# fatchord/WaveRNN

Measured on AMD Instinct MI355X. Metric: audio samples/sec (real-time factor @22.05 kHz), MoL WaveRNN batched generate, higher is better.
Workload: dtype f32

## Files before the change

### wavernn_amd/csrc/wrnn_duo.hip

```cpp
#include <type_traits>

#include "wrnn_ring.h"

namespace wrnn {

#ifndef DUO_XR_FIRST
#define DUO_XR_FIRST 1
#endif

#ifndef DUO_ABLATE
#define DUO_ABLATE 0
#endif
#ifndef DUO_EI_DEPTH
#define DUO_EI_DEPTH 4
#endif

constexpr int DNWGC = 4 * LNJ;
#ifndef DUO_GH_SHIFT
#define DUO_GH_SHIFT 1
#endif
constexpr int DLOGS = 36;
constexpr int DPART = 2 * NW * 3 * 256;
static_assert(O_HOWN == 768 && O_XS == 1024 && O_SP == 1040, "saved state layout");

struct DuoLds {
    int off_h, off_seg, off_xs, off_part, off_log, off_misc, off_prof, off_f3, total;
};
__host__ __device__ inline DuoLds duo_lds(int G)
{
    DuoLds l;
    int o = 0;
    l.off_h = o;    o += G * 256;
    l.off_seg = o;  o += G * 48;
    l.off_xs = o;   o += G * 16;
    l.off_part = o; o += DPART;
    l.off_log = o;  o += SEG * DLOGS;
    l.off_misc = o; o += 2 * LMAXG + 2 * DNWGC;
    l.off_prof = o; o += 2 * 16;
    o = (o + 3) & ~3;
    l.off_f3 = o;   o += SEG * LDC;
    l.total = o;
    return l;
}

#define DPARTOF(q) (PART + (q) * (NW * 3 * 256))
#define PHX(k)                                                                 \
    do {                                                                       \
        if (PROF && tid == 0) {                                                \
            const u64 now_ = __builtin_amdgcn_s_memtime();                     \
            PROFL[k] += now_ - plast;                                          \
            plast = now_;                                                      \
            if (trp && t >= tr_t0 && t < tr_t0 + 3 && ntr < 510)               \
                trp[1 + ntr++] = (now_ << 16) | (u64)(((tri & 15) << 8) | ((k) & 255));   \
        }                                                                      \
    } while (0)
#define TRACE_DECL                                                                                                   \
    u64 *const trp = (PROF && (a.tuning & 16384) && a.prof) ? a.prof + 256 * 32 + (size_t)blockIdx.x * 512 : nullptr; \
    int ntr = 0, tri = 0;                                                                                            \
    const int tr_t0 = a.t0 + (a.t1 - a.t0) / 2;

typedef __attribute__((address_space(3))) void lds_void;
__device__ __forceinline__ void prefetch8(__amdgpu_buffer_rsrc_t rs, float *dst, int voff, int soff)
{
    lds_void *d0 = (lds_void *)dst, *d1 = (lds_void *)(dst + 1024);
    __builtin_amdgcn_raw_ptr_buffer_load_lds(rs, d0, 16, voff, soff, 0, 16 );
    __builtin_amdgcn_raw_ptr_buffer_load_lds(rs, d0, 16, voff, soff, 1024, 16);
    __builtin_amdgcn_raw_ptr_buffer_load_lds(rs, d0, 16, voff, soff, 2048, 16);
    __builtin_amdgcn_raw_ptr_buffer_load_lds(rs, d0, 16, voff, soff, 3072, 16);
    __builtin_amdgcn_raw_ptr_buffer_load_lds(rs, d1, 16, voff + 4096, soff, 0, 16);
    __builtin_amdgcn_raw_ptr_buffer_load_lds(rs, d1, 16, voff + 4096, soff, 1024, 16);
    __builtin_amdgcn_raw_ptr_buffer_load_lds(rs, d1, 16, voff + 4096, soff, 2048, 16);
    __builtin_amdgcn_raw_ptr_buffer_load_lds(rs, d1, 16, voff + 4096, soff, 3072, 16);
}

struct DuoGeo {
    int nact;
    u64 nbpack;
};

template <int MODE, bool LA, bool LP, bool EI, bool PROF>
__device__ __forceinline__ void duo_ih(const LoopArgs &a, float *smem, const int cl, const int J, const int ncl, const bool loc_h, const bool loc_y)
{
    const int G = a.G;
    const DuoLds L = duo_lds(G);
    float *HS = smem + L.off_h, *XS = smem + L.off_xs, *PART = smem + L.off_part;
    int *SEGT = reinterpret_cast<int *>(smem + L.off_seg);
    int *GEO = reinterpret_cast<int *>(smem + L.off_misc);
    u64 *PROFL = reinterpret_cast<u64 *>(smem + L.off_prof);
    u64 plast = 0;
    TRACE_DECL
    const int tid = threadIdx.x, lane = tid & 63, w = __builtin_amdgcn_readfirstlane(tid >> 6);
    const int fi = lane & 15, kq = lane >> 4;
    const int kbase_lane = KCH * w + 4 * kq;
    const int pu = 4 * w + (tid & 3), pj = (tid >> 2) & 15;
    const int prow = LU * J + pu;
    const int T0 = a.t0, T1 = a.t1;
    const int NR = a.Btot, NGR = a.NG;
    unsigned *const status = a.status;
    float *const state = a.state;
    u64 *const profp = a.prof;
    const float *const bhhp = LA ? a.b_hh1 : a.b_hh2;
    const int resume = a.resume, hop = a.hop;
    const int zrow = a.Nall * a.tab_fps;
    constexpr int L_H = LA ? 0 : 1, L_XR = LA ? 5 : 6, L_Y = LA ? 2 : 3, L_GH = LA ? 8 : 12;
    constexpr int L_P0 = LA ? 4 : 5, L_P2 = LA ? 6 : 2;

    float A_ih[3][AF], A_fc[AF];
#pragma unroll
    for (int g = 0; g < 3; ++g) load_afrag(A_ih[g], LA ? a.w_ih1 : a.w_ih2, LA ? H : H + AUX, g * H + LU * J + fi, true, kbase_lane);
    load_afrag(A_fc, LA ? a.fc1_w : a.fc2_w, H + AUX, LU * J + fi, true, kbase_lane);
    float cb_r = 0.f, cb_z = 0.f, cb_n = 0.f, ux_r = 0.f, ux_z = 0.f, ux_n = 0.f, w0o = 0.f;
    if constexpr (LA) {
        cb_r = a.b_ih1[prow]; cb_z = a.b_ih1[H + prow]; cb_n = a.b_ih1[2 * H + prow];
        ux_r = a.u1[prow]; ux_z = a.u1[H + prow]; ux_n = a.u1[2 * H + prow];
        w0o = a.I_w0[prow];
    }

    for (int q = tid; q < L.total; q += NT) smem[q] = 0.f;
    __syncthreads();
    DuoGeo geo;
    geo.nact = 0; geo.nbpack = 0;
    const size_t state_wg = ((size_t)(cl * LNWGC + 2 * J + (LA ? 0 : 1)) * G) * LGRP;
    for (int i = 0; i < G; ++i) {
        const int g = cl + ncl * i;
        if (g >= NGR) break;
        geo.nact = i + 1;
        const int b0 = (int)(((long)g * NR) / NGR), nb = (int)(((long)(g + 1) * NR) / NGR) - b0;
        if (tid == 0) { GEO[2 * i] = a.rb0 + b0; GEO[2 * i + 1] = nb; }
        geo.nbpack |= (u64)(unsigned)nb << (8 * i);
        if (a.resume) {
            const float *sg = a.state + state_wg + (size_t)i * LGRP;
            HS[i * 256 + tid] = sg[O_HOWN + tid];
            if (tid < SEG) XS[i * 16 + tid] = sg[O_XS + tid];
            if (tid < 2 * SEG) SEGT[i * 48 + tid] = reinterpret_cast<const int *>(sg + O_SP)[tid];
        } else if (tid < SEG) {
            const int sc = a.rb0 + b0 + (tid < nb ? tid : nb - 1);
            SEGT[i * 48 + tid] = a.seg_pos[sc];
            SEGT[i * 48 + SEG + tid] = a.seg_lim[sc];
        }
    }
    __syncthreads();
    for (int i = 0; i < geo.nact; ++i) {
        if (tid < SEG) {
            const int nb = (int)((geo.nbpack >> (8 * i)) & 255u);
            const int sc = GEO[2 * i] + (tid < nb ? tid : nb - 1);
            SEGT[i * 48 + 2 * SEG + tid] = sc * a.tab_fps - (SEGT[i * 48 + tid] + a.tab_t0) / a.hop;
        }
    }
    __syncthreads();
    const int nact = geo.nact;
    const u64 nbpack = geo.nbpack;

    const __amdgpu_buffer_rsrc_t xrs = make_rsrc(a.xbuf, (unsigned)(DXBUF_FLOATS * 4));
    const __amdgpu_buffer_rsrc_t crs = make_rsrc(a.c2f, 0x7FFFF000u);
    const __amdgpu_buffer_rsrc_t frs = make_rsrc(LA ? a.c3f : a.c4f, 0x7FFFF000u);
    const int voff_frag = frag_off(w, 0, lane) * 4;
    const int voff_own = (((J * 64) + 16 * w + pj) * 4 + (tid & 3)) * 4;
    const int voff_gh = (256 * (J & 7) + tid) * 16;
    const int cbase = cl * DSLOTB;
    const unsigned magic = a.hop_magic;
    const int mshift = a.hop_shift;

    const int locbits = (loc_h ? 1 : 0) | (loc_y ? 2 : 0);
    const bool late_xo = (a.tuning & 128) == 0, reprobe = (a.tuning & 8) == 0;
    const bool full_chk = !PROF && (a.tuning & 4096) != 0;
    bool dead = false;
    int pp = 0;
    int t = T0;
    int cur = 0;

    struct Carry {
        float c0, c1, c2;
        u32x4 gw;
        unsigned xo, xt;
        int i, pp, t;
    };
    Carry cy;
    cy.c0 = cy.c1 = cy.c2 = 0.f; cy.gw = u32x4{0u, 0u, 0u, 0u}; cy.xo = cy.xt = 0u; cy.i = 0; cy.pp = 0; cy.t = T0;

    auto slot_nb = [&](int i) -> int { return (int)((nbpack >> (8 * i)) & 255u); };

    auto back_gates = [&](const Carry &c) {
        const int bi = c.i, bt = c.t;
        const float *PB = DPARTOF(c.pp);
        const int nb = slot_nb(bi);
        const int sb = cbase + bi * (MAXCL * DSLOTB) + (bt & (DRING - 1)) * XTB;
        const bool live = pj < nb;
        lds_barrier();
        PHX(cur + 1);
        const float pr = get_partial<3>(PB, 0, pu, pj), pz = get_partial<3>(PB, 1, pu, pj), pn = get_partial<3>(PB, 2, pu, pj);
        const float hprev = HS[bi * 256 + tid];
        float ghr, ghz, ghn;
        u32x4 g = c.gw;
        if (bt > T0) {
            const unsigned tag = (unsigned)bt + 1u;
            if (__builtin_expect(__any(live && g.w != tag), 0))
                wait_for([&] { return !__any(live && g.w != tag); },
                         [&] { g = __builtin_amdgcn_raw_buffer_load_b128(xrs, voff_gh, cbase + bi * (MAXCL * DSLOTB) + (L_GH + (J >> 3)) * DLAYERB + (bt & (DGHRING - 1)) * XTB, 16 ); },
                         status, dead, 0x500u | (LA ? 0u : 8u) | 6u, bt);
            ghr = __uint_as_float(g.x); ghz = __uint_as_float(g.y); ghn = __uint_as_float(g.z);
        } else if (resume) {
            const float *sg = state + state_wg + (size_t)bi * LGRP;
            ghr = sg[tid]; ghz = sg[256 + tid]; ghn = sg[512 + tid];
        } else {
            ghr = bhhp[prow]; ghz = bhhp[H + prow]; ghn = bhhp[2 * H + prow];
        }
        float gir, giz, gin, xin;
        unsigned xw = c.xo;
        if (__builtin_expect(__any(live && xw == SENT), 0))
            wait_for([&] { return !__any(live && xw == SENT); },
                     [&] { xw = __builtin_amdgcn_raw_buffer_load_b32(xrs, voff_own, sb + L_P0 * DLAYERB, 16 ); },
                     status, dead, 0x528u, bt);
        if constexpr (LA) {
            float xv;
            if (bt > T0) {
                unsigned xt = c.xt;
                if (__builtin_expect(__any(live && xt == SENT), 0))
                    wait_for([&] { return !__any(live && xt == SENT); },
                             [&] { xt = __builtin_amdgcn_raw_buffer_load_b32(xrs, pj * 4, cbase + bi * (MAXCL * DSLOTB) + 7 * DLAYERB + ((bt - 1) & (DRING - 1)) * XTB, 16 ); },
                             status, dead, 0x520u, bt);
                xv = __uint_as_float(xt);
            } else xv = XS[bi * 16 + pj];
            gir = pr + fmaf(xv, ux_r, cb_r); giz = pz + fmaf(xv, ux_z, cb_z); gin = pn + fmaf(xv, ux_n, cb_n);
            xin = fmaf(w0o, xv, __uint_as_float(xw));
        } else {
            gir = pr + c.c0; giz = pz + c.c1; gin = pn + c.c2;
            xin = __uint_as_float(xw);
        }
        const float hn = (DUO_ABLATE & 16) ? 0.25f * (gir + giz) + 0.1f * (gin + ghr + ghz + ghn) + 0.5f * hprev
                         : MODE == 1 ? gru_update_fast(gir, giz, gin, ghr, ghz, ghn, hprev) : gru_update(gir, giz, gin, ghr, ghz, ghn, hprev);
        HS[bi * 256 + tid] = hn;
        if (DUO_XR_FIRST) publish4l(xrs, sb + L_XR * DLAYERB + J * 1024, tid, xin + hn, live, false);
        publish4l(xrs, sb + L_H * DLAYERB + J * 1024, tid, hn, live, loc_h);
        if (!DUO_XR_FIRST) publish4l(xrs, sb + L_XR * DLAYERB + J * 1024, tid, xin + hn, live, false);
        PHX(cur + 2);
    };
    auto back_relu = [&](const Carry &c) {
        const float *PB = DPARTOF(c.pp);
        const int sb = cbase + c.i * (MAXCL * DSLOTB) + (c.t & (DRING - 1)) * XTB;
        lds_barrier();
        PHX(cur + 1);
        const float yv = fmaxf(get_partial<3>(PB, 0, pu, pj) + c.c0, 0.f);
        publish4l(xrs, sb + L_Y * DLAYERB + J * 1024, tid, yv, pj < slot_nb(c.i), loc_y);
        PHX(cur + 2);
    };

    static_assert(SEG * LDC >= NW * 2048, "the prefetch blocks fit the fc3 region");
    float *const PFW = smem + L.off_f3 + w * 2048;
    auto prefetch_next = [&](auto PHC, int i) {
        constexpr int ph = decltype(PHC)::value;
        const int ring = t & (DRING - 1);
        int nso;
        if constexpr (ph == 0) nso = (i + 1 < nact) ? cbase + (i + 1) * (MAXCL * DSLOTB) + ring * XTB + L_P0 * DLAYERB : cbase + ring * XTB + L_P2 * DLAYERB;
        else nso = (i + 1 < nact) ? cbase + (i + 1) * (MAXCL * DSLOTB) + ring * XTB + L_P2 * DLAYERB
                                  : (t + 1 < T1 ? cbase + ((t + 1) & (DRING - 1)) * XTB + L_P0 * DLAYERB : -1);
        if (nso >= 0) prefetch8(xrs, PFW, voff_frag, nso);
    };
    if constexpr (LP) {
        if (T0 < T1) prefetch8(xrs, PFW, voff_frag, cbase + (T0 & (DRING - 1)) * XTB + L_P0 * DLAYERB);
    }

    auto stage = [&](auto PHC, auto BKC, int i) {
        constexpr int ph = decltype(PHC)::value;
        constexpr int BK = decltype(BKC)::value;
        const int nb = slot_nb(i);
        const int ring = t & (DRING - 1);
        const int sbase = cbase + i * (MAXCL * DSLOTB);
        const int sb = sbase + ring * XTB;
        u32x4 x[8];
        Carry nc;
        nc.c0 = nc.c1 = nc.c2 = 0.f; nc.gw = u32x4{0u, 0u, 0u, 0u}; nc.xo = nc.xt = 0u;
        nc.i = i; nc.pp = pp; nc.t = t;
        if (PROF && tid == 0 && plast == 0) plast = __builtin_amdgcn_s_memtime();
        tri = cy.i;
        if constexpr (LP) {
            asm volatile("s_waitcnt vmcnt(0)" ::: "memory");
#pragma unroll
            for (int r = 0; r < 8; ++r) x[r] = *reinterpret_cast<const u32x4 *>(PFW + r * 256 + lane * 4);
            if (PROF) {
                asm volatile("s_waitcnt lgkmcnt(0)" ::: "memory");
                cur = ph == 0 ? 0 : 8;
                PHX(cur + 0);
            }
        }
        if constexpr (LA && BK == 1) {
            if (reprobe && cy.t > T0)
                cy.xt = __builtin_amdgcn_raw_buffer_load_b32(xrs, pj * 4, cbase + cy.i * (MAXCL * DSLOTB) + 7 * DLAYERB + ((cy.t - 1) & (DRING - 1)) * XTB, 16 );
        }
        if constexpr (!LP && EI) {
            const int so0 = sb + (ph == 0 ? L_P0 : L_P2) * DLAYERB;
#pragma unroll
            for (int r = 0; r < 8; ++r) x[r] = __builtin_amdgcn_raw_buffer_load_b128(xrs, voff_frag + r * 1024, so0, 16 );
        }
        if constexpr (BK == 1) back_gates(cy);
        if constexpr (BK == 2) back_relu(cy);
        cur = ph == 0 ? 0 : 8;
        tri = i;
        int soff_x;
        if constexpr (ph == 0) {
            soff_x = sb + L_P0 * DLAYERB;
            if constexpr (!LP && !EI) {
#pragma unroll
                for (int r = 0; r < 8; ++r) x[r] = ((DUO_ABLATE & 32) && r > 0) ? x[0] : __builtin_amdgcn_raw_buffer_load_b128(xrs, voff_frag + r * 1024, soff_x, 16 );
            }
            if (!late_xo) nc.xo = __builtin_amdgcn_raw_buffer_load_b32(xrs, voff_own, soff_x, 16 );
            if constexpr (LA) {
                if (t > T0) nc.xt = __builtin_amdgcn_raw_buffer_load_b32(xrs, pj * 4, sbase + 7 * DLAYERB + ((t - 1) & (DRING - 1)) * XTB, 16 );
            } else {
                const int fr = table_row(SEGT[i * 48 + pj] + t, SEGT[i * 48 + SEG + pj], SEGT[i * 48 + 2 * SEG + pj], magic, mshift, hop, zrow);
                const int vo = (fr * 3 * H + prow) * 4;
                nc.c0 = __uint_as_float(__builtin_amdgcn_raw_buffer_load_b32(crs, vo, 0, 0));
                nc.c1 = __uint_as_float(__builtin_amdgcn_raw_buffer_load_b32(crs, vo, H * 4, 0));
                nc.c2 = __uint_as_float(__builtin_amdgcn_raw_buffer_load_b32(crs, vo, 2 * H * 4, 0));
            }
            if (t > T0) nc.gw = __builtin_amdgcn_raw_buffer_load_b128(xrs, voff_gh, sbase + (L_GH + (J >> 3)) * DLAYERB + (t & (DGHRING - 1)) * XTB, 16 );
        } else {
            soff_x = sb + L_P2 * DLAYERB;
            if constexpr (!LP && !EI) {
#pragma unroll
                for (int r = 0; r < 8; ++r) x[r] = ((DUO_ABLATE & 32) && r > 0) ? x[0] : __builtin_amdgcn_raw_buffer_load_b128(xrs, voff_frag + r * 1024, soff_x, 16 );
            }
            const int fr = table_row(SEGT[i * 48 + pj] + t, SEGT[i * 48 + SEG + pj], SEGT[i * 48 + 2 * SEG + pj], magic, mshift, hop, zrow);
            nc.c0 = __uint_as_float(__builtin_amdgcn_raw_buffer_load_b32(frs, (fr * H + prow) * 4, 0, 0));
        }
        PHX(cur + 0);
        {
            const bool live = fi < nb;
            const bool there = frag_there(x, live, full_chk);
            if (PROF && tid == 0) { PROFL[cur + 6] += 1; PROFL[cur + 7] += !there; }
            if (__builtin_expect(!there, 0))
                wait_for([&] { return frag_there(x, live, full_chk); },
                         [&] {
#pragma unroll
                             for (int r = 0; r < 8; ++r) x[r] = __builtin_amdgcn_raw_buffer_load_b128(xrs, voff_frag + r * 1024, soff_x, 16 );
                         },
                         status, dead, 0x500u | (LA ? 0u : 8u) | (unsigned)ph, t);
        }
        PHX(cur + 3);
        if (ph == 0 && late_xo) nc.xo = __builtin_amdgcn_raw_buffer_load_b32(xrs, voff_own, soff_x, 16 );
        if (ph == 0 && i == 0) asm volatile("s_waitcnt vmcnt(0)" ::: "memory");
        if (ph == 2 && i == nact - 1) {
            const int which = lane >> 4;
            const int layer = which == 0 ? L_H : (which == 1 ? L_Y : L_XR);
            const bool lloc = ((locbits >> which) & 1) != 0;
            const int vo = layer * DLAYERB + J * 1024 + w * 256 + (lane & 15) * 16;
            const int so = cbase + ((t + DAHEAD_IH) & (DRING - 1)) * XTB;
            const u32x4 q = {SENT, SENT, SENT, SENT};
            if (which < 3) {
#pragma unroll 1
                for (int i2 = 0; i2 < nact; ++i2) {
                    if (lloc) __builtin_amdgcn_raw_buffer_store_b128(q, xrs, vo, so + i2 * (MAXCL * DSLOTB), 0);
                    else __builtin_amdgcn_raw_buffer_store_b128(q, xrs, vo, so + i2 * (MAXCL * DSLOTB), 16 );
                }
            }
        }
        if constexpr (LP) {
            asm volatile("s_waitcnt lgkmcnt(0)" ::: "memory");
            prefetch_next(PHC, i);
        }
        PHX(cur + 4);
        float b[32];
        frag_to_b(x, b);
        float *PW = DPARTOF(pp);
        if constexpr (ph == 0) {
            f32x4 o0, o1, o2;
            if constexpr ((DUO_ABLATE & 8) != 0) { o0 = mfma1(A_ih[0], b); o1 = o0; o2 = o0; }
            else mfma3s(A_ih[0], A_ih[1], A_ih[2], b, o0, o1, o2);
            put_partial<3>(PW, w, 0, lane, o0);
            put_partial<3>(PW, w, 1, lane, o1);
            put_partial<3>(PW, w, 2, lane, o2);
        } else {
            if constexpr ((DUO_ABLATE & 1) != 0) put_partial<3>(PW, w, 0, lane, f32x4{b[0], b[1], b[2], b[3]});
            else put_partial<3>(PW, w, 0, lane, mfma1(A_fc, b));
        }
        PHX(cur + 5);
        cy = nc;
        pp ^= 1;
    };

    using I0 = std::integral_constant<int, 0>;
    using I1 = std::integral_constant<int, 1>;
    using I2 = std::integral_constant<int, 2>;
    for (; t < T1; ++t) {
        if (t == T0) stage(I0{}, I0{}, 0);
        else stage(I0{}, I2{}, 0);
#pragma unroll 1
        for (int i = 1; i < nact; ++i) stage(I0{}, I1{}, i);
        stage(I2{}, I1{}, 0);
#pragma unroll 1
        for (int i = 1; i < nact; ++i) stage(I2{}, I2{}, i);
    }
    cur = 8;
    back_relu(cy);
#pragma unroll 1
    for (int i = 0; i < nact; ++i) {
        const int nb = slot_nb(i);
        const bool live = pj < nb;
        const int sbase = cbase + i * (MAXCL * DSLOTB);
        const int so = sbase + (L_GH + (J >> 3)) * DLAYERB + (T1 & (DGHRING - 1)) * XTB;
        u32x4 gq = __builtin_amdgcn_raw_buffer_load_b128(xrs, voff_gh, so, 16 );
        const unsigned tag = (unsigned)T1 + 1u;
        wait_for([&] { return !__any(live && gq.w != tag); },
                 [&] { gq = __builtin_amdgcn_raw_buffer_load_b128(xrs, voff_gh, so, 16 ); }, status, dead, 0x521u, T1);
        float *sg = state + state_wg + (size_t)i * LGRP;
        sg[tid] = __uint_as_float(gq.x); sg[256 + tid] = __uint_as_float(gq.y); sg[512 + tid] = __uint_as_float(gq.z);
        sg[O_HOWN + tid] = HS[i * 256 + tid];
        if (tid < 2 * SEG) reinterpret_cast<int *>(sg + O_SP)[tid] = SEGT[i * 48 + tid];
        if constexpr (LA) {
            const int sx = sbase + 7 * DLAYERB + ((T1 - 1) & (DRING - 1)) * XTB;
            unsigned v = __builtin_amdgcn_raw_buffer_load_b32(xrs, fi * 4, sx, 16 );
            wait_for([&] { return !__any(fi < nb && v == SENT); },
                     [&] { v = __builtin_amdgcn_raw_buffer_load_b32(xrs, fi * 4, sx, 16 ); }, status, dead, 0x522u, T1);
            if (tid < SEG) sg[O_XS + tid] = (tid < nb) ? __uint_as_float(v) : 0.f;
        }
    }
    if (PROF && tid == 0 && profp) {
        for (int k = 0; k < 16; ++k) profp[(size_t)(blockIdx.x & 255) * 32 + k] += PROFL[k];
        if (trp) trp[0] = (u64)ntr;
    }
}

template <int MODE, bool LA, bool LP, bool PROF>
__device__ __forceinline__ void duo_hh(const LoopArgs &a, float *smem, const int cl, const int J, const int ncl, const bool loc_h)
{
    const int G = a.G;
    const DuoLds L = duo_lds(G);
    float *PART = smem + L.off_part, *LOG = smem + L.off_log, *F3 = smem + L.off_f3;
    int *SEGT = reinterpret_cast<int *>(smem + L.off_seg);
    int *GEO = reinterpret_cast<int *>(smem + L.off_misc);
    u64 *PROFL = reinterpret_cast<u64 *>(smem + L.off_prof);
    u64 plast = 0;
    TRACE_DECL
    int cur = 0;
    const int tid = threadIdx.x, lane = tid & 63, w = __builtin_amdgcn_readfirstlane(tid >> 6);
    const int fi = lane & 15, kq = lane >> 4;
    const int kbase_lane = KCH * w + 4 * kq;
    const int pu = 4 * w + (tid & 3), pj = (tid >> 2) & 15;
    const int prow = LU * J + pu;
    const int T0 = a.t0, T1 = a.t1, C = a.C;
    const int NR = a.Btot, Nall = a.Nall, NGR = a.NG;
    unsigned *const status = a.status;
    u64 *const profp = a.prof;
    float *const outp = a.out, *const dbgl = a.dbg_logits;
    const float *const forcex = a.force_x, *const noise_pre = a.noise_pre, *const fc3f = a.fc3f, *const noise_raw = a.noise;
    constexpr bool MOL = MODE == 1;
    const int Tall = a.T, noise_t0 = a.noise_t0;
    const float *const mels_up = a.mels_up, *const aux_fr = a.aux_fr, *const mel_coef = a.mel_coef;
    const int mel_stage = a.mel_stage;
    const int hop = a.hop;
    const unsigned magic = a.hop_magic;
    const int mshift = a.hop_shift;
    CondTile ct;
    if constexpr (LA) cond_tile_init(ct, a.I_cT, a.I_b, J, lane);
    constexpr int L_H = LA ? 0 : 1, L_GH = LA ? 8 : 12;

    float A_hh[3][AF];
#pragma unroll
    for (int g = 0; g < 3; ++g) load_afrag(A_hh[g], LA ? a.w_hh1 : a.w_hh2, H, g * H + LU * J + fi, true, kbase_lane);

    const float *bhh = LA ? a.b_hh1 : a.b_hh2;
    const float bh_r = bhh[prow], bh_z = bhh[H + prow], bh_n = bhh[2 * H + prow];
    float b3a = 0.f, b3b = 0.f;
    float A_f3[AF];
    if constexpr (!LA) {
        if constexpr (MOL) {
            b3a = a.fc3_b[pu];
            b3b = (16 + pu < 30) ? a.fc3_b[16 + pu] : 0.f;
        } else {
            b3a = a.fc3_b[prow];
            load_afrag(A_f3, a.fc3_w, H, LU * J + fi, true, kbase_lane);
        }
    }

    for (int q = tid; q < L.total; q += NT) smem[q] = 0.f;
    __syncthreads();
    int nact = 0;
// ... 273 lines not shown
                const int h0 = 4 * quad + w;
                float qn[NS][8], lg[NS][8], mx[NS], sum[NS], sum2[NS], best[NS];
                int bidx[NS];
                const size_t tn = (size_t)(t - noise_t0);
#pragma unroll
                for (int s4 = 0; s4 < NS; ++s4) {
                    const int sjc = (h0 + s4 < nb) ? h0 + s4 : nb - 1;
#pragma unroll
                    for (int e = 0; e < 8; ++e) qn[s4][e] = noise_raw[(tn * Nall + b0 + sjc) * C + lane + 64 * e];
                    mx[s4] = -INFINITY;
#pragma unroll
                    for (int e = 0; e < 8; ++e) {
                        lg[s4][e] = LGT[sjc * LDC + lane + 64 * e];
                        mx[s4] = fmaxf(mx[s4], lg[s4][e]);
                    }
                }
                if (dbgl) {
#pragma unroll
                    for (int s4 = 0; s4 < NS; ++s4)
                        if (h0 + s4 < nb)
#pragma unroll
                            for (int e = 0; e < 8; ++e) dbgl[((size_t)t * Nall + b0 + h0 + s4) * C + lane + 64 * e] = lg[s4][e];
                }
#pragma unroll
                for (int s4 = 0; s4 < NS; ++s4) mx[s4] = wave_max64(mx[s4]);
#pragma unroll
                for (int s4 = 0; s4 < NS; ++s4) {
                    sum[s4] = 0.f;
#pragma unroll
                    for (int e = 0; e < 8; ++e) { lg[s4][e] = expf(lg[s4][e] - mx[s4]); sum[s4] += lg[s4][e]; }
                }
#pragma unroll
                for (int s4 = 0; s4 < NS; ++s4) sum[s4] = wave_sum64(sum[s4]);
#pragma unroll
                for (int s4 = 0; s4 < NS; ++s4) {
                    sum2[s4] = 0.f;
#pragma unroll
                    for (int e = 0; e < 8; ++e) { lg[s4][e] = lg[s4][e] / sum[s4]; sum2[s4] += lg[s4][e]; }
                }
#pragma unroll
                for (int s4 = 0; s4 < NS; ++s4) sum2[s4] = wave_sum64(sum2[s4]);
#pragma unroll
                for (int s4 = 0; s4 < NS; ++s4) {
                    best[s4] = -INFINITY;
                    bidx[s4] = 0;
#pragma unroll
                    for (int e = 0; e < 8; ++e) {
                        const float rr = (lg[s4][e] / sum2[s4]) / qn[s4][e];
                        if (rr > best[s4]) { best[s4] = rr; bidx[s4] = lane + 64 * e; }
                    }
                }
#pragma unroll
                for (int s4 = 0; s4 < NS; ++s4) wave_argmax64(best[s4], bidx[s4]);
                if (lane == 0) {
#pragma unroll
                    for (int s4 = 0; s4 < NS; ++s4) {
                        const int sj = h0 + s4;
                        if (sj < nb) {
                            float xv = 2.f * (float)bidx[s4] / ((float)C - 1.f) - 1.f;
                            outp[(size_t)(b0 + sj) * Tall + t] = xv;
                            if (forcex) xv = forcex[(size_t)(b0 + sj) * Tall + t];
                            __builtin_amdgcn_raw_buffer_store_b32(__float_as_uint(xv), xrs, sj * 4, sbase + 7 * DLAYERB + ring * XTB, 16 );
                        }
                    }
                }
            }
            lds_barrier();
#pragma unroll
            for (int r = 0; r < 8; ++r) x[r] = u32x4{0u, 0u, 0u, 0u};
            pend = BK_NONE;
        } else {
            {
                const u32x4 *fp = reinterpret_cast<const u32x4 *>(fc3f + XT + frag_off(w, 0, lane));
#pragma unroll
                for (int r = 0; r < 8; ++r) x[r] = fp[64 * r];
            }
            put_partial<3>(PW, w, 0, lane, mfma1_lds(F3 + frag_off(w, 0, lane), b));
            float4 av1[8];
#pragma unroll
            for (int r = 0; r < 8; ++r) av1[r] = make_float4(__uint_as_float(x[r].x), __uint_as_float(x[r].y), __uint_as_float(x[r].z), __uint_as_float(x[r].w));
            put_partial<3>(PW, w, 1, lane, mfma1_frag(av1, b));
            pend = BK_SAMPLE;
        }
        PHX(cur + 5);
        cy = nc;
        pp ^= 1;
    };

    using K1 = std::integral_constant<int, 1>;
    using K2 = std::integral_constant<int, 2>;
    using K3 = std::integral_constant<int, 3>;
    using K4 = std::integral_constant<int, 4>;
    using BGH = std::integral_constant<int, BK_GH>;
    using BLG = std::integral_constant<int, BK_LG>;
    using BANY = std::integral_constant<int, BK_ANY>;
    cond_step(T0);
    if (T0 + 1 < T1) cond_step(T0 + 1);
    const bool shift = DUO_GH_SHIFT && nact >= 2 && !order1;
    last_here = shift ? nact - 2 : nact - 1;
    if constexpr (order1) {
        for (; t < T1; ++t) {
            if constexpr (LA) {
                if (t + 2 < T1) cond_step(t + 2);
                asm volatile("s_waitcnt vmcnt(0)" ::: "memory");
            }
#pragma unroll 1
            for (int i = 0; i < nact; ++i) {
                stage(K1{}, BANY{}, i);
                if constexpr (!LA) {
                    if (sampler && i == my_slot) stage(K3{}, BGH{}, my_slot);
                }
            }
        }
    } else
    for (; t <= T1; ++t) {
        const bool late = shift && t > T0;
        if (t == T1 && !late) break;
        if constexpr (LA) {
            if (t + 2 < T1) cond_step(t + 2);
            asm volatile("s_waitcnt vmcnt(0)" ::: "memory");
        }
        deferred = late;
        if (late) --t;
        stage(K1{}, BANY{}, late ? nact - 1 : 0);
        if (late) ++t;
        deferred = false;
        if (t == T1) break;
#pragma unroll 1
        for (int i = late ? 0 : 1; i <= last_here; ++i) stage(K1{}, BGH{}, i);
        if constexpr (!LA && MOL) {
            if (sampler) stage(K3{}, BGH{}, my_slot);
        }
        if constexpr (!LA && !MOL) {
            stage(K2{}, BGH{}, 0);
#pragma unroll 1
            for (int i = 1; i < nact; ++i) stage(K2{}, BLG{}, i);
            if (sampler) stage(K4{}, BLG{}, my_slot);
        }
    }
    cur = 0;
    if (pend == BK_GH) back_gh(cy);
    else if (pend == BK_SAMPLE) { if constexpr (!LA && MOL) back_sample(cy); }
    else if (pend == BK_LG) { if constexpr (!LA && !MOL) back_lg(cy); }
    cond_leave();
    if (PROF && tid == 0 && profp) {
        for (int k = 0; k < 16; ++k) profp[(size_t)(blockIdx.x & 255) * 32 + 16 + k] += PROFL[k];
        if (trp) trp[0] = (u64)ntr;
    }
}
#undef DPARTOF
#undef PHX
#undef TRACE_DECL

template <int MODE, bool LP, bool EI, bool PROF>
__global__ __launch_bounds__(NT, 2) void wrnn_duo_kernel(const LoopArgs a)
{
    extern __shared__ __attribute__((aligned(16))) float smem[];
    int cl, wg;
    const int ncl = gridDim.x / DNWGC;
    check_kind(a);
    {
        const int b = blockIdx.x, nblk = gridDim.x;
        if (nblk % 8 == 0 && ncl >= 1 && 8 % ncl == 0) {
            const int xpc = 8 / ncl, per_xcd = nblk / 8;
            const int xcd = b % 8;
            cl = xcd / xpc;
            wg = (xcd % xpc) * per_xcd + b / 8;
        } else {
            cl = b / DNWGC;
            wg = b % DNWGC;
        }
    }
    if (cl >= a.NG) return;
    const int layer = wg / (DNWGC / 2), q = wg % (DNWGC / 2);
    const int hh = q >> 5, J = q & 31;
    bool loc_a = false, loc_b = false;
    {
        int *TAB = reinterpret_cast<int *>(smem) + 2 * LMAXG;
        const int tid = threadIdx.x;
        unsigned *tab = a.xcc_tab + cl * DNWGC;
        if (tid == 0) {
            const unsigned xcc = __builtin_amdgcn_s_getreg((31 << 11) | 20) & 0xFu;
            __hip_atomic_store(tab + wg, xcc + 1u, __ATOMIC_RELAXED, __HIP_MEMORY_SCOPE_AGENT);
            if (!PROF && a.prof && blockIdx.x < 2048 && (a.tuning & 64)) {
                const unsigned hw = __builtin_amdgcn_s_getreg((31 << 11) | 4);
                a.prof[blockIdx.x] = ((u64)xcc << 32) | hw | ((u64)(unsigned)((layer | (hh << 1)) | (J << 2) | (cl << 8)) << 40);
            }
        }
        unsigned v = 1u;
        if (tid < DNWGC) {
            unsigned spins = 0;
            v = ld_agent32(tab + tid);
            while (v == 0u && ++spins < 200000u) {
                __builtin_amdgcn_s_sleep(2);
                v = ld_agent32(tab + tid);
            }
            TAB[tid] = (int)v;
        }
        __syncthreads();
        const int ok_a = (tid < DNWGC / 2) ? (v != 0u && (int)v == TAB[0]) : 1;
        const int ok_b = (tid >= DNWGC / 2 && tid < DNWGC) ? (v != 0u && (int)v == TAB[DNWGC / 2]) : 1;
        loc_a = __syncthreads_and(ok_a) != 0;
        loc_b = __syncthreads_and(ok_b) != 0;
        if (a.tuning & 256) { loc_a = false; loc_b = false; }
        __syncthreads();
    }
#ifndef DUO_ROLES
#define DUO_ROLES 15
#endif
    if (layer == 0) {
        if (hh == 0) { if constexpr ((DUO_ROLES & 1) != 0) duo_ih<MODE, true, LP, EI, PROF>(a, smem, cl, J, ncl, loc_a, false); }
        else { if constexpr ((DUO_ROLES & 2) != 0) duo_hh<MODE, true, LP, PROF>(a, smem, cl, J, ncl, loc_a); }
    } else {
        if (hh == 0) { if constexpr ((DUO_ROLES & 4) != 0) duo_ih<MODE, false, LP, EI, PROF>(a, smem, cl, J, ncl, loc_b, loc_b); }
        else { if constexpr ((DUO_ROLES & 8) != 0) duo_hh<MODE, false, LP, PROF>(a, smem, cl, J, ncl, loc_b); }
    }
}

size_t duo_lds_bytes(int G) { return (size_t)duo_lds(G).total * sizeof(float); }
size_t duo_xbuf_bytes(int G) { return (size_t)G * MAXCL * DNX * DLAYER_ENTRIES * XT * sizeof(float); }
size_t duo_xbuf_bytes_max() { return DXBUF_FLOATS * sizeof(float); }
int duo_max_depth() { return LMAXG; }

hipError_t launch_duo(const LoopArgs &args, int ncl, int mode, hipStream_t stream)
{
    if (ncl < 1 || args.G < 1 || args.G > LMAXG || (mode == 1 && !args.fc3f) || !args.u1 || !args.xcc_tab) return hipErrorInvalidValue;
    const size_t lds = duo_lds_bytes(args.G);
    const bool lp = (args.tuning & 2) != 0;
    const bool ei = !lp && ((args.tuning & 512) ? true : ((args.tuning & 1) ? false : args.G >= DUO_EI_DEPTH));
    const bool prof = mode == 1 && args.prof && !(args.tuning & 64);
    const void *fn = mode == 1 ? (lp ? (prof ? (const void *)wrnn_duo_kernel<1, true, false, true> : (const void *)wrnn_duo_kernel<1, true, false, false>)
                                : ei ? (prof ? (const void *)wrnn_duo_kernel<1, false, true, true> : (const void *)wrnn_duo_kernel<1, false, true, false>)
                                     : (prof ? (const void *)wrnn_duo_kernel<1, false, false, true> : (const void *)wrnn_duo_kernel<1, false, false, false>))
                               : (lp ? (const void *)wrnn_duo_kernel<0, true, false, false> : ei ? (const void *)wrnn_duo_kernel<0, false, true, false> : (const void *)wrnn_duo_kernel<0, false, false, false>);
    hipError_t e = hipFuncSetAttribute(fn, hipFuncAttributeMaxDynamicSharedMemorySize, (int)lds);
    if (e != hipSuccess) return e;
    LoopArgs a = args;
    void *params[] = {(void *)&a};
    return hipLaunchCooperativeKernel(fn, dim3(ncl * DNWGC), dim3(NT), params, (unsigned)lds, stream);
}

}
```

### wavernn_amd/csrc/wrnn_ring.h

```cpp
#pragma once
#include "wrnn_tiles.h"

namespace wrnn {

constexpr int LU = 16;
constexpr int LNJ = H / LU;
constexpr int LNWGC = 2 * LNJ;
constexpr int XT = SEG * H;
constexpr unsigned SENT = 0xFFFFFFFFu;

constexpr int LGRP = 3 * 256 + 256 + 16 + 32 + 32 + 256;
constexpr int O_HOWN = 768, O_XS = 1024, O_SP = 1040, O_FR = 1072, O_XO = 1104;
__device__ __forceinline__ void lds_barrier() { asm volatile("s_waitcnt lgkmcnt(0)\n\ts_barrier" ::: "memory"); }

__device__ __forceinline__ int frag_off(int w, int r, int lane) { return ((w * 8 + r) * 64 + lane) * 4; }

__device__ __forceinline__ void issue(__amdgpu_buffer_rsrc_t rs, int soff, int w, int lane, u32x4 (&x)[8])
{
    const int voff = frag_off(w, 0, lane) * 4;
#pragma unroll
    for (int r = 0; r < 8; ++r) x[r] = __builtin_amdgcn_raw_buffer_load_b128(rs, voff + r * 1024, soff, 16 );
}
__device__ __forceinline__ void issue_sel(__amdgpu_buffer_rsrc_t rs, int soff, int w, int lane, u32x4 (&x)[8], bool on)
{
// ... 184 lines not shown
    const float *lo = (kq == 3) ? aux_row + 4 : mel_row + CK * kq;
    const float *hi = (kq == 2) ? aux_row : lo + 24;
#pragma unroll
    for (int j = 0; j < 7; ++j) {
        v[j] = make_float4(0.f, 0.f, 0.f, 0.f);
        if (valid) v[j] = *reinterpret_cast<const float4 *>(j < 6 ? lo + 4 * j : hi);
    }
}
__device__ __forceinline__ f32x4 cond_mfma(const CondTile &c, const float4 (&v)[7])
{
    f32x4 a0 = {c.bias[0], c.bias[1], c.bias[2], c.bias[3]}, a1 = {0.f, 0.f, 0.f, 0.f};
#pragma unroll
    for (int j = 0; j < 7; ++j) {
        a0 = __builtin_amdgcn_mfma_f32_16x16x4f32(c.w[4 * j + 0], v[j].x, a0, 0, 0, 0);
        a1 = __builtin_amdgcn_mfma_f32_16x16x4f32(c.w[4 * j + 1], v[j].y, a1, 0, 0, 0);
        a0 = __builtin_amdgcn_mfma_f32_16x16x4f32(c.w[4 * j + 2], v[j].z, a0, 0, 0, 0);
        a1 = __builtin_amdgcn_mfma_f32_16x16x4f32(c.w[4 * j + 3], v[j].w, a1, 0, 0, 0);
    }
    return a0 + a1;
}
__device__ __forceinline__ f32x4 cond_tile(const CondTile &c, const float *mel_row, const float *aux_row, bool valid, int lane)
{
    float4 v[7];
    cond_inputs(mel_row, aux_row, valid, lane, v);
    return cond_mfma(c, v);
}

__device__ __forceinline__ void cond_inputs_rows(const float *r0, const float *co, const float *aux_row, bool valid, int lane, float4 (&v)[7])
{
    const int kq = lane >> 4;
#pragma unroll
    for (int j = 0; j < 7; ++j) v[j] = make_float4(0.f, 0.f, 0.f, 0.f);
    if (valid) {
        if (kq == 3) {
#pragma unroll
            for (int j = 0; j < 7; ++j) v[j] = *reinterpret_cast<const float4 *>(aux_row + 4 + 4 * j);
        } else {
            const float c0 = co[0], c1 = co[1], c2 = co[2];
            const float *lo = r0 + CK * kq;
#pragma unroll
            for (int j = 0; j < 7; ++j) {
                if (j == 6 && kq == 2) { v[j] = *reinterpret_cast<const float4 *>(aux_row); continue; }
                const float4 a = *reinterpret_cast<const float4 *>(lo + 4 * j);
                const float4 b = *reinterpret_cast<const float4 *>(lo + MEL + 4 * j);
                const float4 d = *reinterpret_cast<const float4 *>(lo + 2 * MEL + 4 * j);
                v[j] = make_float4(fmaf(c2, d.x, fmaf(c1, b.x, c0 * a.x)), fmaf(c2, d.y, fmaf(c1, b.y, c0 * a.y)),
                                   fmaf(c2, d.z, fmaf(c1, b.z, c0 * a.z)), fmaf(c2, d.w, fmaf(c1, b.w, c0 * a.w)));
            }
        }
    }
}
__device__ __forceinline__ f32x4 cond_tile_rows(const CondTile &c, const float *r0, const float *co, const float *aux_row, bool valid, int lane)
{
    float4 v[7];
    cond_inputs_rows(r0, co, aux_row, valid, lane, v);
    return cond_mfma(c, v);
}

__device__ __forceinline__ float fast_sigmoid(float x) { return __builtin_amdgcn_rcpf(1.0f + __expf(-x)); }
__device__ __forceinline__ float fast_tanh(float x) { return 1.0f - 2.0f * __builtin_amdgcn_rcpf(1.0f + __expf(2.0f * x)); }
__device__ __forceinline__ float gru_update_fast(float gi_r, float gi_z, float gi_n, float gh_r, float gh_z, float gh_n, float h)
{
    const float r = fast_sigmoid(gh_r + gi_r);
    const float z = fast_sigmoid(gh_z + gi_z);
    const float n = fast_tanh(gi_n + gh_n * r);
    return (h - n) * z + n;
}

constexpr int DNX = 17;
constexpr int DRING = 4;
constexpr int DAHEAD_IH = 2;
constexpr int DAHEAD_HH = 3;
constexpr int DGHRING = 2;
constexpr int DLAYER_ENTRIES = DRING;
constexpr size_t DXBUF_FLOATS = (size_t)LMAXG * MAXCL * DNX * DLAYER_ENTRIES * XT;
constexpr int XTB = XT * 4;
constexpr int DLAYERB = DLAYER_ENTRIES * XTB;
constexpr int DSLOTB = DNX * DLAYERB;
static_assert((size_t)LMAXG * MAXCL * DSLOTB < 0x7FFFFFFFull, "32-bit buffer offsets");

__device__ __forceinline__ f32x4 mfma1_frag(const float4 (&av)[8], const float (&b)[32])
{
    f32x4 c0 = {0.f, 0.f, 0.f, 0.f}, c1 = c0;
#pragma unroll
    for (int r = 0; r < 8; r += 2) {
        c0 = __builtin_amdgcn_mfma_f32_16x16x4f32(av[r].x, b[4 * r + 0], c0, 0, 0, 0);
        c1 = __builtin_amdgcn_mfma_f32_16x16x4f32(av[r + 1].x, b[4 * r + 4], c1, 0, 0, 0);
        c0 = __builtin_amdgcn_mfma_f32_16x16x4f32(av[r].y, b[4 * r + 1], c0, 0, 0, 0);
        c1 = __builtin_amdgcn_mfma_f32_16x16x4f32(av[r + 1].y, b[4 * r + 5], c1, 0, 0, 0);
        c0 = __builtin_amdgcn_mfma_f32_16x16x4f32(av[r].z, b[4 * r + 2], c0, 0, 0, 0);
        c1 = __builtin_amdgcn_mfma_f32_16x16x4f32(av[r + 1].z, b[4 * r + 6], c1, 0, 0, 0);
        c0 = __builtin_amdgcn_mfma_f32_16x16x4f32(av[r].w, b[4 * r + 3], c0, 0, 0, 0);
        c1 = __builtin_amdgcn_mfma_f32_16x16x4f32(av[r + 1].w, b[4 * r + 7], c1, 0, 0, 0);
    }
    return c0 + c1;
}

__device__ __forceinline__ void frag_to_b(const u32x4 (&x)[8], float (&b)[32])
{
#pragma unroll
    for (int r = 0; r < 8; ++r) {
        b[4 * r + 0] = __uint_as_float(x[r].x);
        b[4 * r + 1] = __uint_as_float(x[r].y);
        b[4 * r + 2] = __uint_as_float(x[r].z);
        b[4 * r + 3] = __uint_as_float(x[r].w);
    }
}
__device__ __forceinline__ bool frag_there(const u32x4 (&x)[8], bool live)
{
    unsigned m = 0u;
#pragma unroll
    for (int r = 0; r < 8; ++r) m = max(max(m, max(x[r].x, x[r].y)), max(x[r].z, x[r].w));
    return __all(m != SENT || !live);
}

__device__ __forceinline__ bool frag_there(const u32x4 (&x)[8], bool live, bool full)
{
    unsigned m = max(max(max(x[0].w, x[1].w), max(x[2].w, x[3].w)), max(max(x[4].w, x[5].w), max(x[6].w, x[7].w)));
    if (full) {
#pragma unroll
        for (int r = 0; r < 8; ++r) m = max(max(m, x[r].x), max(x[r].y, x[r].z));
    }
    return __all(m != SENT || !live);
}

template <class There, class Reload>
__device__ __forceinline__ void wait_for(There there, Reload reload, unsigned *status, bool &dead, unsigned code, int step)
{
    unsigned spins = 0;
    while (!dead && !there()) {
        if ((++spins & 255u) == 0u) {
            if (ld_agent32(status) != 0u) { dead = true; break; }
            if (spins > SPIN_LIMIT) { report_failure(status, code, blockIdx.x, step, threadIdx.x); dead = true; break; }
        }
        __builtin_amdgcn_s_sleep(1);
        reload();
    }
}

__device__ __forceinline__ void publish4l(__amdgpu_buffer_rsrc_t rs, int soff, int tid, float v, bool on, bool local)
{
    const int iv = __builtin_bit_cast(int, v);
    const int v0 = __builtin_amdgcn_update_dpp(0, iv, 0x00, 0xF, 0xF, true);
    const int v1 = __builtin_amdgcn_update_dpp(0, iv, 0x55, 0xF, 0xF, true);
    const int v2 = __builtin_amdgcn_update_dpp(0, iv, 0xAA, 0xF, 0xF, true);
    const int v3 = __builtin_amdgcn_update_dpp(0, iv, 0xFF, 0xF, 0xF, true);
    if (on && (tid & 3) == 0) {
        const u32x4 q = {(unsigned)v0, (unsigned)v1, (unsigned)v2, (unsigned)v3};
        if (local) __builtin_amdgcn_raw_buffer_store_b128(q, rs, (tid & ~3) * 4, soff, 0);
        else __builtin_amdgcn_raw_buffer_store_b128(q, rs, (tid & ~3) * 4, soff, 16 );
    }
}

__device__ __forceinline__ int table_row(int p, int lim, int tbase, unsigned magic, int shift, int hop, int zrow)
{
    const int q = magic ? (int)(__umulhi((unsigned)p, magic) >> shift) : p / hop;
    return p < lim ? tbase + q : zrow;
}

__device__ __forceinline__ void mfma3s(const float (&a0)[AF], const float (&a1)[AF], const float (&a2)[AF], const float (&b)[32],
                                       f32x4 &o0, f32x4 &o1, f32x4 &o2)
{
    f32x4 c0 = {0.f, 0.f, 0.f, 0.f}, c1 = c0, c2 = c0;
#pragma unroll
    for (int k = 0; k < 32; ++k) {
        c0 = __builtin_amdgcn_mfma_f32_16x16x4f32(a0[k], b[k], c0, 0, 0, 0);
        c1 = __builtin_amdgcn_mfma_f32_16x16x4f32(a1[k], b[k], c1, 0, 0, 0);
        c2 = __builtin_amdgcn_mfma_f32_16x16x4f32(a2[k], b[k], c2, 0, 0, 0);
    }
    o0 = c0; o1 = c1; o2 = c2;
}

__device__ __forceinline__ void mfma_ag(f32x4 &c, float a, float b) { asm("v_mfma_f32_16x16x4_f32 %0, %1, %2, %0" : "+v"(c) : "a"(a), "v"(b)); }
__device__ __forceinline__ f32x4 mfma_ag0(float a, float b)
{
    f32x4 c;
    asm("v_mfma_f32_16x16x4_f32 %0, %1, %2, 0" : "=&v"(c) : "a"(a), "v"(b));
    return c;
}
__device__ __forceinline__ void mfma3s_ag(const float (&a0)[AF], const float (&a1)[AF], const float (&a2)[AF], const float (&b)[32], f32x4 &o0, f32x4 &o1, f32x4 &o2)
{
    f32x4 c0 = mfma_ag0(a0[0], b[0]), c1 = mfma_ag0(a1[0], b[0]), c2 = mfma_ag0(a2[0], b[0]);
#pragma unroll
    for (int k = 1; k < 32; ++k) {
        mfma_ag(c0, a0[k], b[k]);
        mfma_ag(c1, a1[k], b[k]);
        mfma_ag(c2, a2[k], b[k]);
    }
    asm volatile("s_nop 15\n\ts_nop 7" : "+v"(c0), "+v"(c1), "+v"(c2));
    o0 = c0; o1 = c1; o2 = c2;
}
__device__ __forceinline__ f32x4 mfma1_ag(const float (&a)[AF], const float (&b)[32])
{
    f32x4 c0 = mfma_ag0(a[0], b[0]), c1 = mfma_ag0(a[4], b[4]);
#pragma unroll
    for (int r = 0; r < 8; r += 2) {
#pragma unroll
        for (int e = 0; e < 4; ++e) {
            if (r + e > 0) {
                mfma_ag(c0, a[4 * r + e], b[4 * r + e]);
                mfma_ag(c1, a[4 * r + 4 + e], b[4 * r + 4 + e]);
            }
        }
    }
    asm volatile("s_nop 15\n\ts_nop 7" : "+v"(c0), "+v"(c1));
    return c0 + c1;
}

}
```

Measured before the change: 11.20 million.

## Cache conditioning-table rows in LDS and reload only when the hop row changes

Adds a per-slot LDS cache of the conditioning-table values (c2f rows for layer 1 ih, c3f/c4f for the fc stage). A next-change step is computed from the hop and segment limit, then min-reduced across the wave, so the global loads are issued only when some lane's row index changes. This is meant to cut the per-step global loads and table_row arithmetic. In exchange it adds LDS traffic and wave-uniform branching, and it shares the fc3 region, so it cannot be combined with the LDS prefetch path.

```diff
diff --git a/wavernn_amd/csrc/wrnn_duo.hip b/wavernn_amd/csrc/wrnn_duo.hip
--- a/wavernn_amd/csrc/wrnn_duo.hip
+++ b/wavernn_amd/csrc/wrnn_duo.hip
@@ -1,6 +1,7 @@
 #include <type_traits>
 
 #include "wrnn_ring.h"
+#include "wrnn_tabcache.h"
 
 namespace wrnn {
 
@@ -13,6 +14,9 @@
 #endif
 #ifndef DUO_EI_DEPTH
 #define DUO_EI_DEPTH 4
+#endif
+#ifndef DUO_TC_DEPTH
+#define DUO_TC_DEPTH 1
 #endif
 
 constexpr int DNWGC = 4 * LNJ;
@@ -78,7 +82,7 @@
     u64 nbpack;
 };
 
-template <int MODE, bool LA, bool LP, bool EI, bool PROF>
+template <int MODE, bool LA, bool LP, bool EI, bool PROF, bool TCA>
 __device__ __forceinline__ void duo_ih(const LoopArgs &a, float *smem, const int cl, const int J, const int ncl, const bool loc_h, const bool loc_y)
 {
     const int G = a.G;
@@ -164,6 +168,10 @@
     const int locbits = (loc_h ? 1 : 0) | (loc_y ? 2 : 0);
     const bool late_xo = (a.tuning & 128) == 0, reprobe = (a.tuning & 8) == 0;
     const bool full_chk = !PROF && (a.tuning & 4096) != 0;
+    static_assert(!(TCA && LP), "the table cache and the LDS prefetch share the fc3 region");
+    static_assert(SEG * LDC >= LMAXG * NT * 4 + 2 * NW * LMAXG, "the table cache (16 bytes per slot and thread) and its next-change words fit the fc3 region");
+    float *const TC = smem + L.off_f3;
+    int *const TCN = reinterpret_cast<int *>(smem + L.off_f3 + LMAXG * NT * 4);
     bool dead = false;
     int pp = 0;
     int t = T0;
@@ -260,6 +268,22 @@
         if (T0 < T1) prefetch8(xrs, PFW, voff_frag, cbase + (T0 & (DRING - 1)) * XTB + L_P0 * DLAYERB);
     }
 
+    auto lookup_row = [&](int i, int *tcn) -> int {
+        const int pos = SEGT[i * 48 + pj], lim = SEGT[i * 48 + SEG + pj];
+        int q;
+        const int fr = table_row(pos + t, lim, SEGT[i * 48 + 2 * SEG + pj], magic, mshift, hop, zrow, q);
+        if constexpr (TCA) {
+            int nx = table_next_change(t, pos, lim, hop, q);
+            unsigned va, vb;
+            xor_pair_u<4>((unsigned)nx, va, vb);  nx = min((int)va, (int)vb);
+            xor_pair_u<8>((unsigned)nx, va, vb);  nx = min((int)va, (int)vb);
+            xor_pair_u<16>((unsigned)nx, va, vb); nx = min((int)va, (int)vb);
+            xor_pair_u<32>((unsigned)nx, va, vb); nx = min((int)va, (int)vb);
+            *tcn = nx;
+        }
+        return fr;
+    };
+
     auto stage = [&](auto PHC, auto BKC, int i) {
         constexpr int ph = decltype(PHC)::value;
         constexpr int BK = decltype(BKC)::value;
@@ -273,6 +297,10 @@
         nc.i = i; nc.pp = pp; nc.t = t;
         if (PROF && tid == 0 && plast == 0) plast = __builtin_amdgcn_s_memtime();
         tri = cy.i;
+        constexpr bool looks = ph == 2 || !LA;
+        int *const tcn = TCN + ((ph >> 1) * NW + w) * LMAXG + i;
+        int due_at = 0;
+        if constexpr (TCA && looks) due_at = *tcn;
         if constexpr (LP) {
             asm volatile("s_waitcnt vmcnt(0)" ::: "memory");
 #pragma unroll
@@ -306,9 +334,17 @@
             if (!late_xo) nc.xo = __builtin_amdgcn_raw_buffer_load_b32(xrs, voff_own, soff_x, 16 );
             if constexpr (LA) {
                 if (t > T0) nc.xt = __builtin_amdgcn_raw_buffer_load_b32(xrs, pj * 4, sbase + 7 * DLAYERB + ((t - 1) & (DRING - 1)) * XTB, 16 );
+            } else if constexpr (TCA) {
+                float *const e = TC + (i * NT + tid) * 4;
+                if (t >= __builtin_amdgcn_readfirstlane(due_at)) {
+                    const int vo = (lookup_row(i, tcn) * 3 * H + prow) * 4;
+                    e[0] = __uint_as_float(__builtin_amdgcn_raw_buffer_load_b32(crs, vo, 0, 0));
+                    e[1] = __uint_as_float(__builtin_amdgcn_raw_buffer_load_b32(crs, vo, H * 4, 0));
+                    e[2] = __uint_as_float(__builtin_amdgcn_raw_buffer_load_b32(crs, vo, 2 * H * 4, 0));
+                }
+                nc.c0 = e[0]; nc.c1 = e[1]; nc.c2 = e[2];
             } else {
-                const int fr = table_row(SEGT[i * 48 + pj] + t, SEGT[i * 48 + SEG + pj], SEGT[i * 48 + 2 * SEG + pj], magic, mshift, hop, zrow);
-                const int vo = (fr * 3 * H + prow) * 4;
+                const int vo = (lookup_row(i, tcn) * 3 * H + prow) * 4;
                 nc.c0 = __uint_as_float(__builtin_amdgcn_raw_buffer_load_b32(crs, vo, 0, 0));
                 nc.c1 = __uint_as_float(__builtin_amdgcn_raw_buffer_load_b32(crs, vo, H * 4, 0));
                 nc.c2 = __uint_as_float(__builtin_amdgcn_raw_buffer_load_b32(crs, vo, 2 * H * 4, 0));
@@ -320,8 +356,12 @@
 #pragma unroll
                 for (int r = 0; r < 8; ++r) x[r] = ((DUO_ABLATE & 32) && r > 0) ? x[0] : __builtin_amdgcn_raw_buffer_load_b128(xrs, voff_frag + r * 1024, soff_x, 16 );
             }
-            const int fr = table_row(SEGT[i * 48 + pj] + t, SEGT[i * 48 + SEG + pj], SEGT[i * 48 + 2 * SEG + pj], magic, mshift, hop, zrow);
-            nc.c0 = __uint_as_float(__builtin_amdgcn_raw_buffer_load_b32(frs, (fr * H + prow) * 4, 0, 0));
+            if constexpr (TCA) {
+                float *const e = TC + (i * NT + tid) * 4 + 3;
+                if (t >= __builtin_amdgcn_readfirstlane(due_at))
+                    *e = __uint_as_float(__builtin_amdgcn_raw_buffer_load_b32(frs, (lookup_row(i, tcn) * H + prow) * 4, 0, 0));
+                nc.c0 = *e;
+            } else nc.c0 = __uint_as_float(__builtin_amdgcn_raw_buffer_load_b32(frs, (lookup_row(i, tcn) * H + prow) * 4, 0, 0));
         }
         PHX(cur + 0);
         {
@@ -901,7 +941,7 @@
 #undef PHX
 #undef TRACE_DECL
 
-template <int MODE, bool LP, bool EI, bool PROF>
+template <int MODE, bool LP, bool EI, bool PROF, bool TCA>
 __global__ __launch_bounds__(NT, 2) void wrnn_duo_kernel(const LoopArgs a)
 {
     extern __shared__ __attribute__((aligned(16))) float smem[];
@@ -958,10 +998,10 @@
 #define DUO_ROLES 15
 #endif
     if (layer == 0) {
-        if (hh == 0) { if constexpr ((DUO_ROLES & 1) != 0) duo_ih<MODE, true, LP, EI, PROF>(a, smem, cl, J, ncl, loc_a, false); }
+        if (hh == 0) { if constexpr ((DUO_ROLES & 1) != 0) duo_ih<MODE, true, LP, EI, PROF, TCA>(a, smem, cl, J, ncl, loc_a, false); }
         else { if constexpr ((DUO_ROLES & 2) != 0) duo_hh<MODE, true, LP, PROF>(a, smem, cl, J, ncl, loc_a); }
     } else {
-        if (hh == 0) { if constexpr ((DUO_ROLES & 4) != 0) duo_ih<MODE, false, LP, EI, PROF>(a, smem, cl, J, ncl, loc_b, loc_b); }
+        if (hh == 0) { if constexpr ((DUO_ROLES & 4) != 0) duo_ih<MODE, false, LP, EI, PROF, TCA>(a, smem, cl, J, ncl, loc_b, loc_b); }
         else { if constexpr ((DUO_ROLES & 8) != 0) duo_hh<MODE, false, LP, PROF>(a, smem, cl, J, ncl, loc_b); }
     }
 }
@@ -970,6 +1010,14 @@
 size_t duo_xbuf_bytes(int G) { return (size_t)G * MAXCL * DNX * DLAYER_ENTRIES * XT * sizeof(float); }
 size_t duo_xbuf_bytes_max() { return DXBUF_FLOATS * sizeof(float); }
 int duo_max_depth() { return LMAXG; }
+
+template <int MODE, bool PROF>
+static const void *duo_fn(bool lp, bool ei, bool tc)
+{
+    if (lp) return (const void *)wrnn_duo_kernel<MODE, true, false, PROF, false>;
+    if (ei) return tc ? (const void *)wrnn_duo_kernel<MODE, false, true, PROF, true> : (const void *)wrnn_duo_kernel<MODE, false, true, PROF, false>;
+    return tc ? (const void *)wrnn_duo_kernel<MODE, false, false, PROF, true> : (const void *)wrnn_duo_kernel<MODE, false, false, PROF, false>;
+}
 
 hipError_t launch_duo(const LoopArgs &args, int ncl, int mode, hipStream_t stream)
 {
@@ -978,10 +1026,8 @@
     const bool lp = (args.tuning & 2) != 0;
     const bool ei = !lp && ((args.tuning & 512) ? true : ((args.tuning & 1) ? false : args.G >= DUO_EI_DEPTH));
     const bool prof = mode == 1 && args.prof && !(args.tuning & 64);
-    const void *fn = mode == 1 ? (lp ? (prof ? (const void *)wrnn_duo_kernel<1, true, false, true> : (const void *)wrnn_duo_kernel<1, true, false, false>)
-                                : ei ? (prof ? (const void *)wrnn_duo_kernel<1, false, true, true> : (const void *)wrnn_duo_kernel<1, false, true, false>)
-                                     : (prof ? (const void *)wrnn_duo_kernel<1, false, false, true> : (const void *)wrnn_duo_kernel<1, false, false, false>))
-                               : (lp ? (const void *)wrnn_duo_kernel<0, true, false, false> : ei ? (const void *)wrnn_duo_kernel<0, false, true, false> : (const void *)wrnn_duo_kernel<0, false, false, false>);
+    const bool tc = !lp && (args.tuning & 8192) == 0 && args.G >= DUO_TC_DEPTH;
+    const void *fn = mode == 1 ? (prof ? duo_fn<1, true>(lp, ei, tc) : duo_fn<1, false>(lp, ei, tc)) : duo_fn<0, false>(lp, ei, tc);
     hipError_t e = hipFuncSetAttribute(fn, hipFuncAttributeMaxDynamicSharedMemorySize, (int)lds);
     if (e != hipSuccess) return e;
     LoopArgs a = args;
diff --git a/wavernn_amd/csrc/wrnn_ring.h b/wavernn_amd/csrc/wrnn_ring.h
--- a/wavernn_amd/csrc/wrnn_ring.h
+++ b/wavernn_amd/csrc/wrnn_ring.h
@@ -360,10 +360,15 @@
     }
 }
 
+__device__ __forceinline__ int table_row(int p, int lim, int tbase, unsigned magic, int shift, int hop, int zrow, int &q)
+{
+    q = magic ? (int)(__umulhi((unsigned)p, magic) >> shift) : p / hop;
+    return p < lim ? tbase + q : zrow;
+}
 __device__ __forceinline__ int table_row(int p, int lim, int tbase, unsigned magic, int shift, int hop, int zrow)
 {
-    const int q = magic ? (int)(__umulhi((unsigned)p, magic) >> shift) : p / hop;
-    return p < lim ? tbase + q : zrow;
+    int q;
+    return table_row(p, lim, tbase, magic, shift, hop, zrow, q);
 }
 
 __device__ __forceinline__ void mfma3s(const float (&a0)[AF], const float (&a1)[AF], const float (&a2)[AF], const float (&b)[32],
diff --git a/wavernn_amd/csrc/wrnn_tabcache.h b/wavernn_amd/csrc/wrnn_tabcache.h
--- /dev/null
+++ b/wavernn_amd/csrc/wrnn_tabcache.h
@@ -0,0 +1,22 @@
+#pragma once
+
+#if defined(__HIPCC__)
+#define WRNN_TC_HD __host__ __device__
+#else
+#define WRNN_TC_HD
+#endif
+
+namespace wrnn {
+
+constexpr int TAB_NEVER = 0x7FFFFFFF;
+
+WRNN_TC_HD inline int table_next_change(int t, int pos, int lim, int hop, int q)
+{
+    const int p = pos + t;
+    if (p >= lim) return TAB_NEVER;
+    const int at_hop = t + hop - (p - q * hop);
+    const int at_lim = lim - pos;
+    return at_hop < at_lim ? at_hop : at_lim;
+}
+
+}
```

New measurement: 11.13 million. About the same (-0.6%).
